# LepistaBioinformatics/classeq2

Hardware: AMD Instinct MI355X
Metric: query placements/sec, 10k-leaf tree, 150 bp reads (higher is better)
Workload: dtype u64

## Files before the change

classeq2_amd/csrc/cls_api.cpp:

```cpp
#include <hip/hip_runtime.h>
#include <ctype.h>
#include <stdio.h>
#include <stdlib.h>
#include <string.h>

#include <algorithm>
#include <mutex>
#include <new>
#include <string>
#include <thread>
#include <vector>

#include "cls_db.h"
#include "cls_device.h"
#include "cls_kernels.h"
#include "cls_place.h"
#include "cls_tuning.h"

namespace {

thread_local std::string g_err;

int fail(int code, const std::string& msg) {
    g_err = msg;
// ... 7 lines not shown
    } while (0)

struct Workspace {
    uint32_t* ptr = nullptr;
    uint64_t words = 0;
    hipEvent_t done = nullptr;
    hipStream_t stream = nullptr;
    uint64_t seq = 0;
    int launching = 0;
    bool busy = false;
    bool recorded = false;
};
struct TimedPair {
    hipEvent_t t0 = nullptr, t1 = nullptr;
    bool pending = false;
    bool in_use = false;
};
constexpr size_t MAX_WS_SLOTS = 8;
constexpr size_t MAX_TIMED_PAIRS = 256;

struct CallSlot {
    hipStream_t stream = nullptr;
    void *d_bases = nullptr, *d_off = nullptr, *d_out = nullptr, *d_stats = nullptr;
    uint64_t cap_bytes = 0;
    uint32_t cap_reads = 0, cap_stats = 0;
    bool busy = false;
};

cls::PlaceParams resolve(const cls_params* p) {
    cls::PlaceParams r;
    r.max_iterations = (p && (p->flags & CLS_HAS_MAX_ITERATIONS)) ? p->max_iterations : 1000;
    r.remove_intersection = (p && (p->flags & CLS_HAS_REMOVE_INTERSECTION)) ? (p->remove_intersection != 0) : 0;
    double c = 0.7;
    if (p && (p->flags & CLS_HAS_MIN_MATCH_COVERAGE)) {
        c = p->min_match_coverage;
        if (c > 1.0) c = 1.0; else if (c < 0.0) c = 0.0;
    }
    r.min_match_coverage = c;
    return r;
}

}

struct cls_db {
    int device = 0;
    int n_cu = 0;
    cls::DbDev dev{};
    cls_db_info info{};
    void* d_nodes = nullptr;
    void* d_kids = nullptr;
    void* d_table = nullptr;
    void* d_postings = nullptr;
    void* d_postings2 = nullptr;
    void* d_bucket_key = nullptr;
    void* d_mz_bucket = nullptr;
    void* d_direct = nullptr;
    void* d_direct16 = nullptr;
    void* d_sets = nullptr;
    void* d_sets2 = nullptr;
    std::mutex ws_mu;
    uint64_t max_read_len = 0;
    double kernel_ms_sum = 0.0;
    uint64_t kernel_launches = 0;
    std::vector<Workspace> ws;
    std::vector<TimedPair> timed;
    uint64_t ws_seq = 0;
    std::vector<CallSlot> calls;
};

namespace cls {
Tuning& tuning() {
    static Tuning t;
    return t;
}
}
namespace {
struct Knob { const char* name; int cls::Tuning::*field; };
const Knob KNOBS[] = {
    {"no_fast", &cls::Tuning::no_fast}, {"no_order", &cls::Tuning::no_order}, {"force_list", &cls::Tuning::force_list},
    {"no_mask_halves", &cls::Tuning::no_mask_halves}, {"no_fat_direct", &cls::Tuning::no_fat_direct}, {"no_tile", &cls::Tuning::no_tile}, {"tile_pass_codes", &cls::Tuning::tile_pass_codes}, {"tile_set_words", &cls::Tuning::tile_set_words}, {"time_class", &cls::Tuning::time_class}, {"tile_one_per_cu", &cls::Tuning::tile_one_per_cu}, {"tile_min_kmers", &cls::Tuning::tile_min_kmers}, {"no_tile_order", &cls::Tuning::no_tile_order}, {"tile_deal", &cls::Tuning::tile_deal}, {"blocks_per_cu", &cls::Tuning::blocks_per_cu}, {"key_blocks_per_cu", &cls::Tuning::key_blocks_per_cu},
    {"long_blocks_per_cu", &cls::Tuning::long_blocks_per_cu}, {"order_mode", &cls::Tuning::order_mode},
    {"order_windows", &cls::Tuning::order_windows}, {"order_both_strands", &cls::Tuning::order_both_strands},
    {"order_block_shift", &cls::Tuning::order_block_shift}, {"order_sample_shift", &cls::Tuning::order_sample_shift},
    {"profile_stop", &cls::Tuning::profile_stop}, {"timing", &cls::Tuning::timing},
};
}

extern "C" int cls_set_tuning(const char* name, int value) {
    if (!name) return fail(CLS_E_INVALID_ARG, "cls_set_tuning: null name");
    for (const Knob& k : KNOBS)
        if (strcmp(k.name, name) == 0) { cls::tuning().*(k.field) = value; return CLS_OK; }
    return fail(CLS_E_INVALID_ARG, std::string("cls_set_tuning: unknown knob ") + name);
}

extern "C" void cls_tuning_from_env(void) {
    for (const Knob& k : KNOBS) {
        std::string var = "CLS_";
        for (const char* c = k.name; *c; ++c) var += (char)toupper((unsigned char)*c);
        if (const char* v = getenv(var.c_str())) cls::tuning().*(k.field) = *v ? atoi(v) : 1;
    }
}

extern "C" const char* cls_last_error(void) { return g_err.c_str(); }
extern "C" void cls_internal_set_error(const char* msg) { g_err = msg ? msg : ""; }

extern "C" const char* cls_version(void) { return "classeq2_amd 0.1.0 gfx950 abi1"; }

extern "C" int cls_device_count(void) {
    int n = 0;
    if (hipGetDeviceCount(&n) != hipSuccess) return 0;
    return n;
}

extern "C" void cls_db_destroy(cls_db* db) {
    if (!db) return;
    int prev = 0;
    bool have_prev = hipGetDevice(&prev) == hipSuccess;
    (void)hipSetDevice(db->device);
    for (auto& w : db->ws) {
        if (w.done) { if (w.recorded) (void)hipEventSynchronize(w.done); (void)hipEventDestroy(w.done); }
        if (w.ptr) (void)hipFree(w.ptr);
    }
    for (auto& t : db->timed) {
        if (t.t0) (void)hipEventDestroy(t.t0);
        if (t.t1) (void)hipEventDestroy(t.t1);
    }
    for (auto& c : db->calls) {
        if (c.stream) { (void)hipStreamSynchronize(c.stream); (void)hipStreamDestroy(c.stream); }
        for (void* p : {c.d_bases, c.d_off, c.d_out, c.d_stats}) if (p) (void)hipFree(p);
    }
    if (db->d_nodes) (void)hipFree(db->d_nodes);
    if (db->d_kids) (void)hipFree(db->d_kids);
    if (db->d_table) (void)hipFree(db->d_table);
    if (db->d_postings) (void)hipFree(db->d_postings);
    if (db->d_postings2) (void)hipFree(db->d_postings2);
    if (db->d_bucket_key) (void)hipFree(db->d_bucket_key);
    if (db->d_mz_bucket) (void)hipFree(db->d_mz_bucket);
    if (db->d_direct) (void)hipFree(db->d_direct);
    if (db->d_direct16) (void)hipFree(db->d_direct16);
    if (db->d_sets) (void)hipFree(db->d_sets);
    if (db->d_sets2) (void)hipFree(db->d_sets2);
    if (have_prev) (void)hipSetDevice(prev);
    delete db;
}

static int encode(const cls_db_desc* d, cls::EncodedDb& E, const char* who) {
    std::string err;
    int rc = cls::encode_db(d, E, err);
    if (rc != CLS_OK) return fail(rc, std::string(who) + ": " + err);
    if (E.format == cls::FMT_LIST && E.postings.size() >= (1ULL << 32)) return fail(CLS_E_BAD_DB, std::string(who) + ": sorted-list postings exceed 2^32 words");
    return CLS_OK;
}

static int upload(const cls::EncodedDb& E, uint32_t n_buckets, int device, cls_db** out) {
    *out = nullptr;
    int n_dev = 0;
    if (hipGetDeviceCount(&n_dev) != hipSuccess || n_dev == 0)
        return fail(CLS_E_NO_DEVICE, "cls_db_create: no HIP device is visible (the placement path has no CPU fallback)");
    if (device < 0) CLS_HIP(hipGetDevice(&device));
    if (device >= n_dev) return fail(CLS_E_INVALID_ARG, "cls_db_create: device ordinal out of range");
    CLS_HIP(hipSetDevice(device));
    hipDeviceProp_t prop;
    CLS_HIP(hipGetDeviceProperties(&prop, device));
    cls_db* db = new cls_db();
    db->device = device;
    db->n_cu = prop.multiProcessorCount;
// ... 697 lines not shown
```

classeq2_amd/csrc/cls_devutil.h:

```cpp
#pragma once
#include <hip/hip_runtime.h>
#include <stdint.h>

#include "cls_device.h"
#include "cls_murmur.h"

namespace cls {
namespace {

__device__ __forceinline__ void wave_sync() {
    __builtin_amdgcn_fence(__ATOMIC_RELEASE, "wavefront");
    __builtin_amdgcn_wave_barrier();
    __builtin_amdgcn_fence(__ATOMIC_ACQUIRE, "wavefront");
}

__device__ __forceinline__ uint32_t uniform(uint32_t v) { return __builtin_amdgcn_readfirstlane(v); }

__device__ __forceinline__ uint32_t wave_sum(uint32_t v) {
    v += (uint32_t)__builtin_amdgcn_update_dpp(0, (int)v, 0xb1, 0xf, 0xf, true);
    v += (uint32_t)__builtin_amdgcn_update_dpp(0, (int)v, 0x4e, 0xf, 0xf, true);
    v += (uint32_t)__builtin_amdgcn_update_dpp(0, (int)v, 0x114, 0xf, 0xf, true);
    v += (uint32_t)__builtin_amdgcn_update_dpp(0, (int)v, 0x118, 0xf, 0xf, true);
    v += (uint32_t)__builtin_amdgcn_update_dpp(0, (int)v, 0x142, 0xa, 0xf, true);
    v += (uint32_t)__builtin_amdgcn_update_dpp(0, (int)v, 0x143, 0xc, 0xf, true);
    return (uint32_t)__builtin_amdgcn_readlane((int)v, 63);
}

struct snode_t { uint32_t s[8]; };
__device__ __forceinline__ snode_t load_node(const DNode* nodes, uint32_t row) {
    typedef __attribute__((address_space(4))) const uint32_t as4_u32;
    typedef __attribute__((address_space(4))) const char as4_char;
    as4_u32* p = (as4_u32*)((as4_char*)(uintptr_t)nodes + (uint32_t)(__builtin_amdgcn_readfirstlane(row) * (uint32_t)sizeof(DNode)));
    snode_t r;
#pragma unroll
    for (int i = 0; i < 8; ++i) r.s[i] = p[i];
    return r;
}

struct snode_pair_t { uint32_t s[16]; };
__device__ __forceinline__ snode_pair_t load_node_pair(const DNode* nodes, uint32_t row) {
    typedef __attribute__((address_space(4))) const uint32_t as4_u32;
    as4_u32* p = (as4_u32*)(uintptr_t)(nodes + __builtin_amdgcn_readfirstlane(row));
    snode_pair_t r;
#pragma unroll
    for (int i = 0; i < 16; ++i) r.s[i] = p[i];
    return r;
}

template <class T, bool ADDR32>
__device__ __forceinline__ T ldx(const void* base, uint32_t index) {
    if constexpr (ADDR32) return *reinterpret_cast<const T*>(reinterpret_cast<const char*>(base) + (uint32_t)(index * (uint32_t)sizeof(T)));
    else return reinterpret_cast<const T*>(base)[index];
}

template <bool ADDR32>
__device__ __forceinline__ uint2 ld_half(const uint32_t* half, uint32_t x, uint32_t right) {
    if constexpr (ADDR32) return ldx<uint2, true>(half, 2 * x + right);
    else return reinterpret_cast<const uint2*>(half)[2ull * x + right];
}

__device__ __forceinline__ uint64_t lds_u64(const uint8_t* p) { uint64_t v; __builtin_memcpy(&v, p, 8); return v; }
__device__ __forceinline__ uint64_t murmur3_h1_lds(const uint8_t* p, uint32_t len) {
    Mur3 m;
    const uint32_t nblocks = len >> 4;
#pragma unroll 1
    for (uint32_t b = 0; b < nblocks; ++b) m.block(lds_u64(p + 16 * b), lds_u64(p + 16 * b + 8));
    const uint32_t t = len & 15u;
    const uint8_t* tail = p + 16 * nblocks;
    uint64_t k1 = 0, k2 = 0;
    if (t > 0) { k1 = lds_u64(tail); if (t < 8) k1 &= (1ull << (8 * t)) - 1; }
    if (t > 8) { k2 = lds_u64(tail + 8) & ((1ull << (8 * (t - 8))) - 1); }
    return m.finish(k1, k2, t, len);
}

__device__ __forceinline__ uint32_t lds_prefix_code(const uint8_t* p, uint32_t m) {
    uint64_t x = (lds_u64(p) >> 1) & 0x0303030303030303ull;
    x = (x | (x >> 6)) & 0x000F000F000F000Full;
    x = (x | (x >> 12)) & 0x000000FF000000FFull;
    x = (x | (x >> 24)) & 0xFFFFull;
    return (uint32_t)x & ((1u << (2 * m)) - 1u);
}

__device__ __forceinline__ uint32_t mix32(uint32_t x) {
    x ^= x >> 16; x *= 0x7feb352du; x ^= x >> 15; x *= 0x846ca68bu; x ^= x >> 16;
    return x;
}

}
}
```

classeq2_amd/csrc/cls_kernels.hip:

```cpp
#include <hip/hip_runtime.h>
#include <stdlib.h>

#include <algorithm>
#include <type_traits>

#include "cls_device.h"
#include "cls_devutil.h"
#include "cls_kernels.h"
#include "cls_murmur.h"
#include "cls_sort.h"
#include "cls_tuning.h"

namespace cls {

namespace {

constexpr int WAVES_PER_BLOCK = 4;
#ifndef MIN_WAVES_PER_EU
#define MIN_WAVES_PER_EU 4
#endif
#ifndef FAST_MIN_WAVES
#define FAST_MIN_WAVES 5
#endif
#ifndef CLS_NARROW_CANON_BITS
// ... 1585 lines not shown
        const uint64_t b0 = have ? offsets[r] : 0, L64 = have ? offsets[r + 1] - b0 : 0;
        const bool keyed = have && L64 >= k && 2 * (L64 - k + 1) <= (uint64_t)key_cap;
        const uint32_t L = keyed ? (uint32_t)std::min<uint64_t>(L64, 64 + k - 1) : 0, nf = keyed ? L - k + 1 : 0;
        bool bad = false;
        for (uint32_t i = hl; i < L; i += 32) {
            uint8_t c = bases[b0 + i];
            if (c >= 'a' && c <= 'z') c -= 32;
            bad |= !(c == 'A' || c == 'C' || c == 'G' || c == 'T');
            ascii[i] = c;
        }
        const bool ok = keyed && half_of(__ballot(bad)) == 0;
        wave_sync();
        for (uint32_t w = hl; w < (L + 15) / 16 + 1; w += 32) {
            uint32_t acc = 0;
#pragma unroll
            for (int q = 0; q < 4; ++q) {
                uint32_t t = *reinterpret_cast<const uint32_t*>(ascii + 16 * w + 4 * q);
                t = (t >> 1) & 0x03030303u;
                t = (t | (t >> 6) | (t >> 12) | (t >> 18)) & 0xFFu;
                acc |= t << (8 * q);
            }
            if (w < WORDS) packed[w] = acc;
        }
        wave_sync();
        uint32_t e[2], hs[2];
#pragma unroll
        for (int s = 0; s < 2; ++s) {
            const uint32_t p = hl + 32 * s;
            const bool valid = ok && p < nf;
            const uint32_t w = valid ? p >> 4 : 0, sh = valid ? (2 * p) & 31 : 0;
            const uint32_t d0 = packed[w], d1 = packed[w + 1];
            uint32_t code = (uint32_t)((((uint64_t)d1 << 32) | d0) >> sh) & kmask;
            uint32_t rcc = __builtin_bitreverse32(code ^ (0xAAAAAAAAu & kmask));
            rcc = ((rcc >> 1) & 0x55555555u) | ((rcc & 0x55555555u) << 1);
            rcc >>= (32 - 2 * k);
            code = rcc < code ? rcc : code;
            const uint32_t v = ldx<uint32_t, ADDR32>(direct, valid ? code : 0u);
            e[s] = valid ? v : 0u;
            hs[s] = mix32(code);
        }
        uint32_t cand = 0, n_cand = 0;
        for (uint32_t tier = 0; tier < 4; ++tier) {
            const bool need = n_cand < 4;
            uint32_t c_new = 0, n_new = 0;
#pragma unroll
            for (int s = 0; s < 2; ++s) {
                const bool c = (e[s] & SET_ID_MASK) != 0 && (e[s] >> TIER_SHIFT) <= tier;
                c_new |= (c ? 1u : 0u) << s;
                n_new += (uint32_t)__popc(half_of(__ballot(c)));
            }
            if (need) { cand = c_new; n_cand = n_new; }
            if (__ballot(n_cand < 4) == 0) break;
        }
        uint32_t rank = n_cand >> 1, prefix = 0;
        for (int bit = (int)db.set_bits - 1; bit >= 0; --bit) {
            uint32_t c0 = 0;
#pragma unroll
            for (int s = 0; s < 2; ++s) {
                const uint32_t t = e[s] & SET_ID_MASK;
                const bool z = ((cand >> s) & 1u) && ((t ^ prefix) >> (bit + 1)) == 0 && !((t >> bit) & 1u);
                c0 += (uint32_t)__popc(half_of(__ballot(z)));
            }
            if (rank >= c0) { rank -= c0; prefix |= 1u << bit; }
        }
        uint32_t mh = 0xFFFFFFFFu, mha = 0xFFFFFFFFu;
#pragma unroll
        for (int s = 0; s < 2; ++s) {
            if ((cand >> s) & 1u) mh = hs[s] < mh ? hs[s] : mh;
            if ((e[s] & SET_ID_MASK) != 0) mha = hs[s] < mha ? hs[s] : mha;
        }
        for (int o = 16; o > 0; o >>= 1) {
            const uint32_t o1 = __shfl_xor(mh, o), o2 = __shfl_xor(mha, o);
            mh = o1 < mh ? o1 : mh;
            mha = o2 < mha ? o2 : mha;
        }
        if (have && hl == 0) {
            keys[r] = (ok && n_cand) ? make_order_key(key_mode, prefix, mh, mha, block_shift, db.set_bits) : ~0ull;
            idx[r] = r;
        }
        wave_sync();
    }
}

constexpr int LONG_THREADS = 256;
constexpr int LONG_STATE_WORDS = 5;

constexpr uint32_t LONG_LDS_ARITY = 256;
struct LongSh {
    uint32_t acc[4];
    unsigned long long acc64;
    uint32_t n_next;
    uint32_t n_pass, n_best, best_row;
    int32_t best_diff, best_one, best_rest;
    uint32_t cpre[LONG_LDS_ARITY + 1];
    uint32_t cnt_l[LONG_LDS_ARITY], only_l[LONG_LDS_ARITY];
};

__device__ __forceinline__ uint32_t append_slot(bool keep, uint32_t* counter) {
    const uint32_t lane = threadIdx.x & 63;
    const uint64_t m = __ballot(keep);
    if (!m) return 0;
    const int leader = __ffsll((unsigned long long)m) - 1;
    uint32_t base = 0;
    if ((int)lane == leader) base = atomicAdd(counter, (uint32_t)__popcll(m));
    base = __shfl(base, leader);
    return base + (uint32_t)__popcll(m & ((1ull << lane) - 1));
}

template <int N>
__device__ __forceinline__ void long_sum(uint32_t (&v)[N], LongSh& sh) {
    __syncthreads();
    if (threadIdx.x < N) sh.acc[threadIdx.x] = 0;
    __syncthreads();
#pragma unroll
    for (int i = 0; i < N; ++i) {
        const uint32_t w = wave_sum(v[i]);
        if ((threadIdx.x & 63) == 0 && w) atomicAdd(&sh.acc[i], w);
    }
    __syncthreads();
#pragma unroll
    for (int i = 0; i < N; ++i) v[i] = sh.acc[i];
}

template <bool SPLIT, bool STATS>
__global__ __launch_bounds__(LONG_THREADS) void place_long_kernel(DbDev db, PlaceParams prm, const uint8_t* __restrict__ bases,
                                                                  const uint64_t* __restrict__ offsets,
                                                                  const uint32_t* __restrict__ list,
                                                                  const uint32_t* __restrict__ list_len,
                                                                  cls_placement* __restrict__ out, cls_query_stats* __restrict__ stats,
                                                                  uint32_t* __restrict__ ws, uint64_t ws_stride_words, uint32_t cap,
                                                                  uint32_t set_size, uint32_t arity_pad) {
    __shared__ LongSh sh;
    constexpr uint32_t NT = LONG_THREADS;
    const uint32_t tid = threadIdx.x, lane = tid & 63;
    uint32_t* const buf0 = ws + (size_t)blockIdx.x * ws_stride_words;
    uint32_t* const buf1 = buf0 + (size_t)LONG_STATE_WORDS * cap;
    uint32_t* const cnt = buf1 + (size_t)LONG_STATE_WORDS * cap;
    uint32_t* const only = cnt + arity_pad;
    uint32_t* const set = buf1;
    uint32_t* const ent = buf0 + 4 * (size_t)cap;
    const DNode* __restrict__ nodes = db.nodes;
    const uint32_t* __restrict__ post = db.postings;
    const uint4* __restrict__ recs = reinterpret_cast<const uint4*>(db.postings);
    const uint32_t k = db.k, m_eff = db.m_eff;
    const bool rm = prm.remove_intersection != 0;
    const uint32_t n_list = *list_len;
    for (uint32_t li = blockIdx.x; li < n_list; li += gridDim.x) {
        __syncthreads();
        const uint32_t r = list[li];
        const uint64_t b0 = offsets[r], L64 = offsets[r + 1] - b0;
        auto put_stats = [&](uint32_t nk_, uint32_t nm, uint32_t nr, uint64_t lp) {
            if (STATS && stats && tid == 0) {
                uint64_t* s = reinterpret_cast<uint64_t*>(stats + r);
                s[0] = (uint64_t)nk_ | ((uint64_t)nm << 32);
                s[1] = (uint64_t)nr;
                s[2] = lp;
            }
        };
        auto record = [&](uint32_t status, int32_t one, int32_t rest, uint32_t levels, uint64_t clade) {
            if (tid == 0) {
                uint64_t* o = reinterpret_cast<uint64_t*>(out + r);
                o[0] = (uint64_t)(status & 0xFF) | ((uint64_t)(uint32_t)one << 32);
                o[1] = (uint64_t)(uint32_t)rest | ((uint64_t)levels << 32);
                o[2] = clade;
            }
        };
// ... 263 lines not shown
                            st[0] = lo; st[1] = hi; st[2] = vlo; st[3] = vhi; st[4] = cur[4 * (size_t)cap + j];
                        }
                    }
                }
                const uint32_t p = append_slot(keep, &sh.n_next);
                if (keep) {
#pragma unroll
                    for (int i = 0; i < (SPLIT ? 3 : LONG_STATE_WORDS); ++i) nxt[(size_t)i * cap + p] = st[i];
                }
            }
            __syncthreads();
            n_act = sh.n_next;
            { uint32_t* t = cur; cur = nxt; nxt = t; }
            prow = best_row;
        }
    }
}

constexpr int CLASSIFY_THREADS = 256, CLASSIFY_PER_THREAD = 4;
struct ClassCaps { uint32_t cap[N_LISTS]; };
__global__ __launch_bounds__(CLASSIFY_THREADS) void classify_kernel(const uint64_t* __restrict__ offsets, const uint32_t* __restrict__ order, uint32_t n_reads, uint32_t k, ClassCaps caps,
                                                                   uint32_t* __restrict__ lists, uint32_t* __restrict__ counts,
                                                                   cls_placement* __restrict__ out, cls_query_stats* __restrict__ stats) {
    __shared__ uint32_t s_cnt[N_LISTS], s_base[N_LISTS];
    if (threadIdx.x < N_LISTS) s_cnt[threadIdx.x] = 0;
    __syncthreads();
    const uint32_t lane = threadIdx.x & 63;
    const uint32_t first = blockIdx.x * (CLASSIFY_THREADS * CLASSIFY_PER_THREAD) + threadIdx.x;
    int cls_id[CLASSIFY_PER_THREAD];
    uint32_t pos[CLASSIFY_PER_THREAD], rd[CLASSIFY_PER_THREAD];
#pragma unroll
    for (int i = 0; i < CLASSIFY_PER_THREAD; ++i) {
        const uint32_t at = first + i * CLASSIFY_THREADS;
        const uint32_t r = (order && at < n_reads) ? order[at] : at;
        rd[i] = r;
        cls_id[i] = -1;
        pos[i] = 0;
        if (at < n_reads) {
            const uint64_t L = offsets[r + 1] - offsets[r];
            const uint64_t nk = L < k ? 0 : 2 * (L - k + 1);
#pragma unroll
            for (int c = N_LISTS - 1; c >= 0; --c) if (nk <= caps.cap[c]) cls_id[i] = c;
            if (cls_id[i] < 0) {
                uint64_t* o = reinterpret_cast<uint64_t*>(out + r);
                o[0] = CLS_ERR_READ_TOO_LONG; o[1] = 0; o[2] = 0;
                if (stats) {
                    uint64_t* st = reinterpret_cast<uint64_t*>(stats + r);
                    st[0] = nk > 0xFFFFFFFFull ? 0xFFFFFFFFull : nk; st[1] = 0; st[2] = 0;
                }
            }
        }
#pragma unroll
        for (int c = 0; c < N_LISTS; ++c) {
            const uint64_t m = __ballot(cls_id[i] == c);
            if (!m) continue;
            uint32_t base = 0;
            if (lane == 0) base = atomicAdd(&s_cnt[c], (uint32_t)__popcll(m));
            base = __shfl(base, 0);
            if (cls_id[i] == c) pos[i] = base + (uint32_t)__popcll(m & ((1ull << lane) - 1));
        }
    }
    __syncthreads();
    if (threadIdx.x < N_LISTS) s_base[threadIdx.x] = s_cnt[threadIdx.x] ? atomicAdd(&counts[threadIdx.x], s_cnt[threadIdx.x]) : 0u;
    __syncthreads();
#pragma unroll
    for (int i = 0; i < CLASSIFY_PER_THREAD; ++i) {
        const int c = cls_id[i];
        if (c >= 0) lists[(size_t)c * n_reads + s_base[c] + pos[i]] = rd[i];
    }
}

}

namespace {
constexpr int N_CLASSES = 2;
constexpr int BLK_WAVES = 8, BLK_SLOTS = 16, BLK_SET_BITS = 14;
constexpr int ORDER_KEY_BITS_MAX = TIER_SHIFT + 20;
int order_key_bits(const DbDev& db) {
    const Tuning& tn = tuning();
    const int bits = tn.order_mode == 1 ? (int)db.set_bits + 20 : std::max(1, (int)db.set_bits - tn.order_block_shift) + 16;
    return std::min<int>(64, bits + 1);
}
constexpr int CLS_SLOTS[N_CLASSES] = {5, 16};
constexpr int CLS_SET_BITS[N_CLASSES] = {9, 11};
constexpr int NARROW_CANON_BITS = CLS_NARROW_CANON_BITS;

bool use_fast(const DbDev& db);
bool use_order(const DbDev& db, uint32_t n_reads) {
    return use_fast(db) && !tuning().no_order && n_reads >= 4096;
}
bool use_fast(const DbDev& db) {
    const bool front = db.direct != nullptr || (db.addr32 && db.k <= 256);
    return db.format == FMT_SPLIT && (db.binary_tree || db.max_nonleaf_arity <= FAST_MAX_ARITY) && front && !tuning().no_fast;
}
int fast_mode(const DbDev& db) { return db.direct == nullptr ? 2 : (db.direct16 && db.addr32) ? (db.canonical ? 4 : 3) : db.canonical ? 1 : 0; }
bool mode_canonical(int mode) { return mode == 1 || mode == 4; }
int set_bits_of(const DbDev& db, int c) { return (c == 0 && use_fast(db) && mode_canonical(fast_mode(db))) ? NARROW_CANON_BITS : CLS_SET_BITS[c]; }
uint32_t seq_cap_of(const DbDev& db, int c) { return (2 * (64 * CLS_SLOTS[c] / 2 + db.k) + 15) & ~15u; }
uint32_t ascii_cap_of(const DbDev& db, int c) {
    const uint32_t fwd = 64 * CLS_SLOTS[c] / 2 + db.k + 16;
    return ((db.direct ? fwd : 2 * fwd) + 15) & ~15u;
}
uint32_t child_ws_stride(const DbDev& db);
constexpr uint32_t CHILD_LDS_MAX = 256;
bool child_in_lds(const DbDev& db) { return child_ws_stride(db) != 0 && child_ws_stride(db) <= CHILD_LDS_MAX; }
size_t smem_of(const DbDev& db, int c) {
    if (use_fast(db)) {
        const uint32_t ac = ascii_cap_of(db, c);
        const uint32_t packed = db.direct ? 4u * (((ac >> 4) + 2 + 3) & ~3u) : 0u;
        return (size_t)WAVES_PER_BLOCK * (ac + packed + (12u << set_bits_of(db, c)) + (db.binary_tree ? 0u : 12u * FAST_MAX_ARITY + 16u));
    }
    return (size_t)WAVES_PER_BLOCK * (seq_cap_of(db, c) + (4u << CLS_SET_BITS[c]) + 4u * 64 * CLS_SLOTS[c]) +
           (child_in_lds(db) ? (size_t)WAVES_PER_BLOCK * 2 * child_ws_stride(db) * 4 : 0);
}

using FastFn = decltype(place_fast_kernel<CLS_SLOTS[0], CLS_SET_BITS[0], false, false, 0, false>);
using SplitFn = decltype(place_split_kernel<CLS_SLOTS[0], CLS_SET_BITS[0], false, false>);
using WaveFn = decltype(place_wave_kernel<CLS_SLOTS[0], CLS_SET_BITS[0], false, false>);
struct ClassKernel {
    FastFn* fast;
    SplitFn* split;
    WaveFn* wave;
    size_t smem;
    std::string name;
    const void* fn() const { return fast ? (const void*)fast : split ? (const void*)split : (const void*)wave; }
};
template <int SLOTS, int SET_BITS>
ClassKernel class_kernel_t(const DbDev& db, int c, bool stats) {
    const size_t smem = smem_of(db, c);
    auto fast = [&](auto... v) { return ClassKernel{place_fast_kernel<decltype(v)::value...>, nullptr, nullptr, smem, instance_name("place_fast_kernel", v...)}; };
    auto split = [&](auto... v) { return ClassKernel{nullptr, place_split_kernel<decltype(v)::value...>, nullptr, smem, instance_name("place_split_kernel", v...)}; };
    auto wave = [&](auto... v) { return ClassKernel{nullptr, nullptr, place_wave_kernel<decltype(v)::value...>, smem, instance_name("place_wave_kernel", v...)}; };
    const Int<SLOTS> sl;
    const Int<SET_BITS> sb;
    return with_bool(stats, [&](auto st) {
        if (use_fast(db)) {
            return with_bool(!db.binary_tree, [&](auto poly) {
                const std::true_type addr32;
                switch (fast_mode(db)) {
                    case 2: return fast(sl, sb, st, addr32, Int<2>{}, poly);
                    case 3: return fast(sl, sb, st, addr32, Int<3>{}, poly);
                    case 4: return fast(sl, sb, st, addr32, Int<4>{}, poly);
                }
                return with_bool(db.addr32, [&](auto a32) { return fast_mode(db) == 1 ? fast(sl, sb, st, a32, Int<1>{}, poly) : fast(sl, sb, st, a32, Int<0>{}, poly); });
            });
        }
        if (db.format == FMT_SPLIT) return with_bool(!db.binary_tree, [&](auto poly) { return split(sl, sb, st, poly); });
        return with_bool(db.max_nonleaf_arity <= 2, [&](auto binary) { return wave(sl, sb, st, binary); });
    });
}
ClassKernel class_kernel(const DbDev& db, int c, bool stats) {
    if (c == 1) return class_kernel_t<CLS_SLOTS[1], CLS_SET_BITS[1]>(db, 1, stats);
    if (set_bits_of(db, 0) != CLS_SET_BITS[0]) return class_kernel_t<CLS_SLOTS[0], NARROW_CANON_BITS>(db, 0, stats);
    return class_kernel_t<CLS_SLOTS[0], CLS_SET_BITS[0]>(db, 0, stats);
}

uint32_t child_ws_stride(const DbDev& db) {
    if (db.format == FMT_SPLIT) return db.binary_tree ? 0u : ((std::max(db.max_nonleaf_arity, 1u) + 63) & ~63u);
    return db.max_nonleaf_arity <= 2 ? 0u : ((db.max_nonleaf_arity + 63) & ~63u);
}
uint32_t blk_seq_cap(const DbDev& db) { return (2 * (64 * BLK_WAVES * BLK_SLOTS / 2 + db.k) + 15) & ~15u; }
auto block_kernel(const DbDev& db, bool stats) {
    const size_t smem = (size_t)blk_seq_cap(db) + (4u << BLK_SET_BITS) + 4u * 64 * BLK_WAVES * BLK_SLOTS + 64 +
                        (child_in_lds(db) ? (size_t)2 * child_ws_stride(db) * 4 : 0);
    auto inst = [&](auto... v) { return pick(place_block_kernel<decltype(v)::value...>, smem, "place_block_kernel", v...); };
    const bool split = db.format == FMT_SPLIT, binary = split ? db.binary_tree != 0 : db.max_nonleaf_arity <= 2;
    return with_bool(stats, [&](auto st) { return with_bool(binary, [&](auto bi) { return with_bool(split, [&](auto sp) {
        return inst(Int<BLK_WAVES>{}, Int<BLK_SLOTS>{}, Int<BLK_SET_BITS>{}, st, bi, sp);
    }); }); });
}
auto long_kernel(const DbDev& db, bool stats) {
    auto inst = [&](auto... v) { return pick(place_long_kernel<decltype(v)::value...>, 0, "place_long_kernel", v...); };
    return with_bool(db.format == FMT_SPLIT, [&](auto sp) { return with_bool(stats, [&](auto st) { return inst(sp, st); }); });
}

using KeyFn = decltype(order_key_kernel<2, true, true, false>);
using KeyHalfFn = decltype(order_key_half_kernel<true>);
struct KeyKernel {
    KeyFn* full;
    KeyHalfFn* half;
    size_t smem;
    std::string name;
    const void* fn() const { return full ? (const void*)full : (const void*)half; }
};
KeyKernel key_kernel(const DbDev& db, bool sizing) {
    const Tuning& tn = tuning();
    const bool fwd = !tn.order_both_strands, hashed = fast_mode(db) == 2;
    if (!sizing && !hashed && fwd && tn.order_windows == 64 && (uint32_t)tn.order_sample_shift >= 32)
        return with_bool(db.addr32, [&](auto a32) { return KeyKernel{nullptr, order_key_half_kernel<decltype(a32)::value>, 0, instance_name("order_key_half_kernel", a32)}; });
    const uint32_t ac = ascii_cap_of(db, 0);
    const size_t smem = (size_t)WAVES_PER_BLOCK * (ac + (db.direct ? 4u * (((ac >> 4) + 2 + 3) & ~3u) : 0u) + 16u);
    auto inst = [&](auto... v) { return KeyKernel{order_key_kernel<decltype(v)::value...>, nullptr, smem, instance_name("order_key_kernel", v...)}; };
    auto of = [&](auto a32, auto hs) {
        if (fwd && tn.order_windows <= 64) return inst(Int<2>{}, a32, std::true_type{}, hs);
        if (fwd || sizing) return inst(Int<CLS_SLOTS[0]>{}, a32, std::true_type{}, hs);
        return inst(Int<CLS_SLOTS[0]>{}, a32, std::false_type{}, hs);
    };
    if (hashed) return of(std::true_type{}, std::true_type{});
    return db.addr32 ? of(std::true_type{}, std::false_type{}) : of(std::false_type{}, std::false_type{});
}
}

void PlacePlan::class_caps(uint32_t (&cap)[N_LISTS]) const {
    for (uint32_t& c : cap) c = 0;
    cap[0] = (uint32_t)(64 * CLS_SLOTS[0]);
    if (max_kmers > cap[0]) cap[1] = (uint32_t)(64 * CLS_SLOTS[1]);
    if (max_kmers > (uint32_t)(64 * CLS_SLOTS[1])) cap[2] = tiled ? tile_from : (uint32_t)(64 * BLK_WAVES * BLK_SLOTS);
    if (tiled) {
        for (uint32_t i = 0; i < tile.n_sub; ++i) cap[3 + i] = tile.sub[i].cap_kmers;
        cap[6] = tile.whole.cap_kmers;
    }
    cap[7] = long_cap;
}

std::string PlacePlan::class_kernel_name(const DbDev& db, int c, bool stats) const {
    if (c < 2) return class_kernel(db, c, stats).name;
    if (c == 2) return block_kernel(db, stats).name;
    if (c < 6) return tile_kernel_name(db, stats, tile.sub[c - 3]);
    if (c == 6) return tile_kernel_name(db, stats, tile.whole);
    return long_kernel(db, stats).name;
}

PlacePlan plan_place(const DbDev& db, uint32_t n_reads, uint32_t n_cu, bool stats, uint32_t long_cap, uint32_t n_long) {
    PlacePlan p{};
    const int forced = tuning().blocks_per_cu;
    const uint32_t want = (n_reads + WAVES_PER_BLOCK - 1) / WAVES_PER_BLOCK;
    uint64_t child_words = 0;
    for (int c = 0; c < N_CLASSES; ++c) {
        int per_cu = forced;
        const ClassKernel k = class_kernel(db, c, stats);
        if (per_cu <= 0 && (hipOccupancyMaxActiveBlocksPerMultiprocessor(&per_cu, k.fn(), 64 * WAVES_PER_BLOCK, k.smem) != hipSuccess || per_cu <= 0))
            per_cu = 1;
        uint32_t cap = n_cu * (uint32_t)per_cu;
        if (child_ws_stride(db) && !child_in_lds(db)) {
            const uint64_t per_block = (uint64_t)WAVES_PER_BLOCK * 2 * child_ws_stride(db) * 4;
            const uint64_t fit = std::max<uint64_t>(1, (128ull << 20) / per_block);
            if (cap > fit) cap = (uint32_t)fit;
        }
        p.grid[c] = want < cap ? (want ? want : 1) : cap;
        if (!child_in_lds(db)) child_words = std::max<uint64_t>(child_words, (uint64_t)p.grid[c] * WAVES_PER_BLOCK * 2 * child_ws_stride(db));
    }
    p.grid_blk = std::max<uint32_t>(1, std::min<uint32_t>(n_reads, n_cu));
    if (!child_in_lds(db)) child_words = std::max<uint64_t>(child_words, (uint64_t)p.grid_blk * 2 * child_ws_stride(db));
    p.ordered = use_order(db, n_reads);
    uint64_t w = 16 + (uint64_t)N_LISTS * n_reads;
    w += w & 1;
    if (p.ordered) {
        p.grid[0] = std::max<uint32_t>(8, p.grid[0] & ~7u);
        p.grid[1] = std::max<uint32_t>(8, p.grid[1] & ~7u);
        {
            int per_cu = tuning().key_blocks_per_cu;
            const KeyKernel k = key_kernel(db, true);
            if (per_cu <= 0 && (hipOccupancyMaxActiveBlocksPerMultiprocessor(&per_cu, k.fn(), 64 * WAVES_PER_BLOCK, k.smem) != hipSuccess || per_cu <= 0)) per_cu = 4;
            if (tuning().key_blocks_per_cu <= 0 && fast_mode(db) == 2) per_cu *= 2;
            p.grid_key = std::max<uint32_t>(1, std::min<uint32_t>(want, n_cu * (uint32_t)per_cu));
        }
        p.keys_off_words = w;
        w += 6 * (uint64_t)n_reads;
        p.sort_off_words = w;
        p.sort_bytes = order_temp_bytes(n_reads);
        w += (p.sort_bytes + 3) / 4 + 2;
        w += w & 1;
    }
    p.child_off_words = w;
    w += child_words;
    w += w & 1;
    p.max_kmers = n_long ? std::max<uint32_t>(long_cap, 2u) : MAX_READ_KMERS;
    const uint32_t blk_cap = (uint32_t)(64 * BLK_WAVES * BLK_SLOTS);
    p.tile_from = blk_cap;
    if (tile_usable(db)) {
        p.tile_from = tuning().tile_min_kmers > 0 ? std::min<uint32_t>(blk_cap, (uint32_t)tuning().tile_min_kmers) : (uint32_t)(64 * CLS_SLOTS[1]);
        if (p.max_kmers > p.tile_from) {
            p.tile = tile_plan(db, stats, p.tile_from, p.max_kmers, n_reads, n_cu);
            p.tiled = p.tile.whole.cap_kmers > p.tile_from;
        }
    }
    if (p.tiled) {
        p.tile_off_words = w;
        w += p.tile.scratch_words;
        w += w & 1;
    } else p.tile_from = blk_cap;
    if (p.max_kmers > MAX_READ_KMERS || p.tiled) {
        long_cap = p.max_kmers;
        p.long_cap = long_cap;
        p.long_set = 1;
        while (p.long_set < 2 * (uint64_t)long_cap) p.long_set <<= 1;
        p.long_arity = (std::max(db.max_nonleaf_arity, 1u) + 63) & ~63u;
        p.long_stride_words = 2 * (uint64_t)LONG_STATE_WORDS * long_cap + 2 * (uint64_t)p.long_arity;
        const uint64_t fit = std::max<uint64_t>(1, (2ull << 30) / (p.long_stride_words * 4));
        const uint64_t per_cu_long = (uint64_t)std::max(1, tuning().long_blocks_per_cu);
        p.grid_long = (uint32_t)std::min<uint64_t>({(uint64_t)std::max<uint32_t>(1u, n_long ? n_long : n_reads), (uint64_t)n_cu * per_cu_long, fit});
        if (p.tiled && p.tile.whole.cap_kmers >= long_cap) p.grid_long = std::min<uint32_t>(p.grid_long, 8u);
        p.long_off_words = w;
        w += p.long_stride_words * p.grid_long;
    }
    p.ws_bytes = w * 4;
    p.blk = p.max_kmers > (uint32_t)(64 * CLS_SLOTS[1]) && (!p.tiled || p.tile_from > (uint32_t)(64 * CLS_SLOTS[1]));
    const bool gene = tuning().time_class == 2;
    p.timed = p.tiled && (p.max_kmers > MAX_READ_KMERS || gene) ? PlacePlan::TIME_TILE : p.blk && gene ? PlacePlan::TIME_BLOCK : PlacePlan::TIME_CLASS0;
    p.timed_name = p.timed == PlacePlan::TIME_TILE ? p.tile.name : p.timed == PlacePlan::TIME_BLOCK ? block_kernel(db, stats).name : class_kernel(db, 0, stats).name;
    return p;
}

hipError_t launch_place(const DbDev& db, const PlaceParams& prm, const PlacePlan& plan, const uint8_t* d_bases,
                        const uint64_t* d_offsets, uint32_t n_reads, cls_placement* d_out, cls_query_stats* d_stats,
                        uint32_t* d_ws, hipStream_t stream, hipEvent_t ev_start, hipEvent_t ev_stop) {
    if (n_reads == 0) return hipSuccess;
    uint32_t* counts = d_ws;
    uint32_t* lists[N_LISTS];
    for (int c = 0; c < N_LISTS; ++c) lists[c] = d_ws + 16 + (size_t)c * n_reads;
    uint32_t* child_ws = (child_ws_stride(db) && !child_in_lds(db)) ? d_ws + plan.child_off_words : nullptr;
    hipError_t e = hipMemsetAsync(counts, 0, 64, stream);
    if (e != hipSuccess) return e;
    const uint32_t profile_stop = (uint32_t)tuning().profile_stop;
    const uint32_t ws_stride = child_ws_stride(db);
    const bool st = d_stats != nullptr;
    auto classify = [&](const uint32_t* order) {
        ClassCaps caps{};
        plan.class_caps(caps.cap);
        return launch_kernel(classify_kernel, dim3((n_reads + CLASSIFY_THREADS * CLASSIFY_PER_THREAD - 1) / (CLASSIFY_THREADS * CLASSIFY_PER_THREAD)), dim3(CLASSIFY_THREADS), 0,
                             stream, d_offsets, order, n_reads, db.k, caps, lists[0], counts, d_out, d_stats);
    };
    const uint32_t* list0 = lists[0];
    uint32_t list0_n = 0, xcd_chunks = 0;
    if (!plan.ordered) e = classify(nullptr);
    else {
        uint64_t* keys_in = reinterpret_cast<uint64_t*>(d_ws + plan.keys_off_words);
        uint64_t* keys_out = keys_in + n_reads;
        uint32_t* idx_in = reinterpret_cast<uint32_t*>(keys_out + n_reads);
        uint32_t* idx_out = idx_in + n_reads;
        const Tuning& tn = tuning();
        const uint32_t key_mode = (uint32_t)tn.order_mode;
        const uint32_t block_shift = (uint32_t)tn.order_block_shift;
        const uint32_t key_cap = (plan.tiled && !tn.no_tile_order) ? 0xFFFFFFFFu : (uint32_t)(64 * CLS_SLOTS[1]);
        const KeyKernel k = key_kernel(db, false);
        const dim3 block(64 * WAVES_PER_BLOCK);
        if (k.half) {
            const uint32_t grid_half = std::max<uint32_t>(1, std::min<uint32_t>((n_reads + 2 * WAVES_PER_BLOCK - 1) / (2 * WAVES_PER_BLOCK), plan.grid_key));
            e = launch_kernel(k.half, dim3(grid_half), block, k.smem, stream, db, d_bases, d_offsets, n_reads, keys_in, idx_in, key_mode, block_shift, key_cap);
        } else {
            e = launch_kernel(k.full, dim3(plan.grid_key), block, k.smem, stream, db, d_bases, d_offsets, n_reads, keys_in, idx_in, ascii_cap_of(db, 0), key_mode,
                              block_shift, (uint32_t)tn.order_sample_shift, tn.order_both_strands ? 0u : 1u, key_cap);
        }
        if (e != hipSuccess) return e;
        e = order_reads(d_ws + plan.sort_off_words, keys_in, idx_out, n_reads, order_key_bits(db) - 1, stream);
        if (e != hipSuccess) return e;
        list0 = idx_out;
        list0_n = n_reads;
        xcd_chunks = 1;
        e = classify(idx_out);
    }
    if (e != hipSuccess) return e;
    auto launch_class = [&](int c) {
        const ClassKernel k = class_kernel(db, c, st);
        const dim3 grid(plan.grid[c]), block(64 * WAVES_PER_BLOCK);
        if (k.fast) {
            return launch_kernel(k.fast, grid, block, k.smem, stream, db, prm, d_bases, d_offsets, xcd_chunks ? list0 : lists[c], counts + c, list0_n, xcd_chunks,
                                 d_out, d_stats, ascii_cap_of(db, c), profile_stop);
        }
        if (k.split)
            return launch_kernel(k.split, grid, block, k.smem, stream, db, prm, d_bases, d_offsets, lists[c], counts + c, d_out, d_stats, seq_cap_of(db, c),
                                 profile_stop, child_ws, ws_stride);
        return launch_kernel(k.wave, grid, block, k.smem, stream, db, prm, d_bases, d_offsets, lists[c], counts + c, d_out, d_stats, seq_cap_of(db, c), child_ws,
                             ws_stride);
    };
    auto timed = [&](PlacePlan::Timed t, auto&& launch) {
        if (ev_start && plan.timed == t) (void)hipEventRecord(ev_start, stream);
        const hipError_t r = launch();
        if (ev_stop && plan.timed == t) (void)hipEventRecord(ev_stop, stream);
        return r;
    };
    e = timed(PlacePlan::TIME_CLASS0, [&] { return launch_class(0); });
    if (e != hipSuccess) return e;
    if (plan.max_kmers > (uint32_t)(64 * CLS_SLOTS[0])) {
        e = launch_class(1);
        if (e != hipSuccess) return e;
    }
    if (plan.blk) {
        const auto k = block_kernel(db, st);
        e = timed(PlacePlan::TIME_BLOCK, [&] {
            return launch_kernel(k.fn, dim3(plan.grid_blk), dim3(64 * BLK_WAVES), k.smem, stream, db, prm, d_bases, d_offsets, lists[2], counts + 2, d_out, d_stats,
                                 blk_seq_cap(db), child_ws, ws_stride);
        });
        if (e != hipSuccess) return e;
    }
    if (plan.tiled) {
        const uint32_t* sub_lists[TILE_MAX_SUB] = {lists[3], lists[4], lists[5]};
        const uint32_t* sub_lens[TILE_MAX_SUB] = {counts + 3, counts + 4, counts + 5};
        e = timed(PlacePlan::TIME_TILE, [&] {
            return tile_launch(db, prm, plan.tile, st, d_bases, d_offsets, sub_lists, sub_lens, lists[6], counts + 6, d_out, d_stats, lists[7], counts + 7,
                               d_ws + plan.tile_off_words, plan.ordered && !tuning().no_tile_order, stream);
        });
        if (e != hipSuccess) return e;
    }
    if (plan.grid_long) {
        const auto k = long_kernel(db, st);
        e = launch_kernel(k.fn, dim3(plan.grid_long), dim3(LONG_THREADS), k.smem, stream, db, prm, d_bases, d_offsets, lists[7], counts + 7, d_out, d_stats,
                          d_ws + plan.long_off_words, plan.long_stride_words, plan.long_cap, (uint32_t)plan.long_set, plan.long_arity);
    }
    return e;
}

}
```

classeq2_amd/csrc/cls_tuning.h:

```cpp
#pragma once

namespace cls {

struct Tuning {
    int no_fast = 0;
    int no_order = 0;
    int force_list = 0;
    int no_mask_halves = 0;
    int no_fat_direct = 0;
    int no_tile = 0;
    int tile_pass_codes = 0;
    int tile_set_words = 0;
    int tile_min_kmers = 0;
    int tile_deal = 64;
    int no_tile_order = 0;
    int tile_one_per_cu = 0;
    int time_class = 0;
    int blocks_per_cu = 0;
    int key_blocks_per_cu = 0;
    int long_blocks_per_cu = 2;
    int order_mode = 0;
    int order_windows = 64;
    int order_both_strands = 0;
    int order_block_shift = 2;
    int order_sample_shift = 32;
    int profile_stop = 0;
    int timing = 0;
};

Tuning& tuning();

}
```

Baseline: 157.7 million.

## Add bottom-k hash-sampled order-key kernel with four reads per wave

Adds a new order-key kernel that packs each read into shared memory with one read per 16-lane quarter-wave. It hashes every canonical k-mer window with an invertible mix and selects the n smallest hashes (bottom-k, default 16) by repeated row-level DPP min reductions. Only the sampled k-mers are looked up in the direct table, and the codes are recovered with unmix32, so fewer random table gathers are needed per read and four reads share each wave. Sort keys now come from a sample, which may change read ordering and locality in the classify stage. The sampling loop adds serial reduction work per read.

```diff
diff --git a/classeq2_amd/csrc/cls_api.cpp b/classeq2_amd/csrc/cls_api.cpp
--- a/classeq2_amd/csrc/cls_api.cpp
+++ b/classeq2_amd/csrc/cls_api.cpp
@@ -113,6 +113,7 @@
     {"long_blocks_per_cu", &cls::Tuning::long_blocks_per_cu}, {"order_mode", &cls::Tuning::order_mode},
     {"order_windows", &cls::Tuning::order_windows}, {"order_both_strands", &cls::Tuning::order_both_strands},
     {"order_block_shift", &cls::Tuning::order_block_shift}, {"order_sample_shift", &cls::Tuning::order_sample_shift},
+    {"order_sample", &cls::Tuning::order_sample},
     {"profile_stop", &cls::Tuning::profile_stop}, {"timing", &cls::Tuning::timing},
 };
 }
diff --git a/classeq2_amd/csrc/cls_devutil.h b/classeq2_amd/csrc/cls_devutil.h
--- a/classeq2_amd/csrc/cls_devutil.h
+++ b/classeq2_amd/csrc/cls_devutil.h
@@ -24,6 +24,13 @@
     v += (uint32_t)__builtin_amdgcn_update_dpp(0, (int)v, 0x142, 0xa, 0xf, true);
     v += (uint32_t)__builtin_amdgcn_update_dpp(0, (int)v, 0x143, 0xc, 0xf, true);
     return (uint32_t)__builtin_amdgcn_readlane((int)v, 63);
+}
+
+__device__ __forceinline__ uint32_t row16_min(uint32_t v) {
+    v = min(v, (uint32_t)__builtin_amdgcn_update_dpp(0, (int)v, 0xB1, 0xF, 0xF, false));
+    v = min(v, (uint32_t)__builtin_amdgcn_update_dpp(0, (int)v, 0x4E, 0xF, 0xF, false));
+    v = min(v, (uint32_t)__builtin_amdgcn_update_dpp(0, (int)v, 0x141, 0xF, 0xF, false));
+    return min(v, (uint32_t)__builtin_amdgcn_update_dpp(0, (int)v, 0x140, 0xF, 0xF, false));
 }
 
 struct snode_t { uint32_t s[8]; };
@@ -85,6 +92,10 @@
     x ^= x >> 16; x *= 0x7feb352du; x ^= x >> 15; x *= 0x846ca68bu; x ^= x >> 16;
     return x;
 }
+__device__ __forceinline__ uint32_t unmix32(uint32_t x) {
+    x ^= x >> 16; x *= 0x43021123u; x ^= (x >> 15) ^ (x >> 30); x *= 0x1d69e2a5u; x ^= x >> 16;
+    return x;
+}
 
 }
 }
diff --git a/classeq2_amd/csrc/cls_kernels.hip b/classeq2_amd/csrc/cls_kernels.hip
--- a/classeq2_amd/csrc/cls_kernels.hip
+++ b/classeq2_amd/csrc/cls_kernels.hip
@@ -1691,6 +1691,148 @@
     }
 }
 
+constexpr uint32_t SAMPLE_MAX_WINDOWS = 160;
+constexpr uint32_t SAMPLE_MAX = 64;
+__device__ __forceinline__ uint32_t nonzero_bytes(uint32_t v) { return (((v & 0x7F7F7F7Fu) + 0x7F7F7F7Fu) | v) & 0x80808080u; }
+template <bool ADDR32>
+__global__ __launch_bounds__(64 * WAVES_PER_BLOCK) void order_key_sample_kernel(DbDev db, const uint8_t* __restrict__ bases,
+                                                                              const uint64_t* __restrict__ offsets, uint32_t n_reads,
+                                                                              uint64_t* __restrict__ keys, uint32_t* __restrict__ idx,
+                                                                              uint32_t key_mode, uint32_t block_shift, uint32_t key_cap,
+                                                                              uint32_t n_sample) {
+    constexpr uint32_t PER = SAMPLE_MAX_WINDOWS / 16;
+    constexpr uint32_t SL = SAMPLE_MAX / 16;
+    constexpr uint32_t MAXL = SAMPLE_MAX_WINDOWS + DIRECT_MAX_K - 1;
+    constexpr uint32_t WORDS = (MAXL + 15) / 16 + 1;
+    static_assert(WORDS <= 16 && SAMPLE_MAX_WINDOWS % 16 == 0 && SAMPLE_MAX % 16 == 0, "one packed word per lane");
+    __shared__ uint32_t s_packed[WAVES_PER_BLOCK * 4][WORDS];
+    const uint32_t wave = threadIdx.x >> 6, lane = threadIdx.x & 63, quarter = lane >> 4, ql = lane & 15;
+    uint32_t* packed = s_packed[wave * 4 + quarter];
+    const uint32_t k = db.k;
+    const uint32_t kmask = (1u << (2 * k)) - 1u;
+    const uint32_t* __restrict__ direct = db.direct;
+    const uint32_t r_first = (blockIdx.x * WAVES_PER_BLOCK + wave) * 4, stride = gridDim.x * WAVES_PER_BLOCK * 4;
+    auto mine = [&](uint64_t m) { return (uint32_t)(m >> (16 * quarter)) & 0xFFFFu; };
+    auto canon_at = [&](uint32_t p) {
+        const uint32_t w = p >> 4, sh = (2 * p) & 31;
+        const uint32_t code = (uint32_t)((((uint64_t)packed[w + 1] << 32) | packed[w]) >> sh) & kmask;
+        uint32_t rcc = __builtin_bitreverse32(code ^ (0xAAAAAAAAu & kmask));
+        rcc = ((rcc >> 1) & 0x55555555u) | ((rcc & 0x55555555u) << 1);
+        rcc >>= (32 - 2 * k);
+        return rcc < code ? rcc : code;
+    };
+    for (uint32_t r0 = r_first; r0 < n_reads; r0 += stride) {
+        const uint32_t r = r0 + quarter;
+        const bool have = r < n_reads;
+        const uint64_t b0 = have ? offsets[r] : 0, L64 = have ? offsets[r + 1] - b0 : 0;
+        const bool keyed = have && L64 >= k && 2 * (L64 - k + 1) <= (uint64_t)key_cap;
+        const bool sampled = keyed && L64 - k + 1 <= SAMPLE_MAX_WINDOWS;
+        const uint32_t nf = keyed ? (sampled ? (uint32_t)(L64 - k + 1) : 64u) : 0u, L = keyed ? nf + k - 1 : 0u;
+        bool bad = false;
+        if (keyed && ql < (L + 15) / 16 + 1) {
+            const uint8_t* p = bases + b0 + 16 * ql;
+            const uintptr_t a = (uintptr_t)p & ~(uintptr_t)3, end = (uintptr_t)(bases + b0 + L);
+            const uint32_t sh = 8u * ((uint32_t)(uintptr_t)p & 3u);
+            uint32_t d[5];
+#pragma unroll
+            for (int i = 0; i < 5; ++i) d[i] = a + 4 * i < end ? *reinterpret_cast<const uint32_t*>(a + 4 * i) : 0u;
+            uint32_t acc = 0;
+#pragma unroll
+            for (int q = 0; q < 4; ++q) {
+                uint32_t t = (uint32_t)((((uint64_t)d[q + 1] << 32) | d[q]) >> sh);
+                const int left = (int)L - (int)(16 * ql + 4 * q);
+                const uint32_t in = left >= 4 ? 0xFFFFFFFFu : left <= 0 ? 0u : (1u << (8 * left)) - 1u;
+                const uint32_t lc = t | 0x20202020u;
+                bad |= (nonzero_bytes(lc ^ 0x61616161u) & nonzero_bytes(lc ^ 0x63636363u) & nonzero_bytes(lc ^ 0x67676767u) &
+                        nonzero_bytes(lc ^ 0x74747474u) & in) != 0;
+                t = (t >> 1) & 0x03030303u;
+                t = (t | (t >> 6) | (t >> 12) | (t >> 18)) & 0xFFu;
+                acc |= t << (8 * q);
+            }
+            packed[ql] = acc;
+        }
+        const bool ok = keyed && mine(__ballot(bad)) == 0;
+        wave_sync();
+        uint32_t pick[SL];
+#pragma unroll
+        for (int s = 0; s < (int)SL; ++s) pick[s] = 0xFFFFFFFFu;
+        const bool any_sampled = __ballot(ok && sampled) != 0;
+        if (any_sampled) {
+            uint32_t h[PER];
+#pragma unroll
+            for (int j = 0; j < (int)PER; ++j) {
+                const uint32_t p = ql + 16 * j;
+                const bool valid = ok && sampled && p < nf;
+                h[j] = valid ? mix32(canon_at(valid ? p : 0u)) : 0xFFFFFFFFu;
+            }
+            uint32_t lo = 0;
+            for (uint32_t i = 0; i < n_sample; ++i) {
+                uint32_t m = 0xFFFFFFFFu;
+#pragma unroll
+                for (int j = 0; j < (int)PER; ++j) m = min(m, h[j] >= lo ? h[j] : 0xFFFFFFFFu);
+                m = row16_min(m);
+#pragma unroll
+                for (int s = 0; s < (int)SL; ++s)
+                    if (i == 16 * s + ql) pick[s] = m;
+                lo = m == 0xFFFFFFFFu ? m : m + 1;
+                if (__ballot(m != 0xFFFFFFFFu) == 0) break;
+            }
+        }
+        const uint32_t n_slots = __ballot(ok && !sampled) ? SL : (n_sample + 15) / 16;
+        uint32_t e[SL], hs[SL];
+#pragma unroll
+        for (int s = 0; s < (int)SL; ++s) {
+            e[s] = 0;
+            hs[s] = 0xFFFFFFFFu;
+            if ((uint32_t)s >= n_slots) continue;
+            const uint32_t p = ql + 16 * s;
+            const bool valid = ok && (sampled ? pick[s] != 0xFFFFFFFFu : p < nf);
+            const uint32_t code = sampled ? unmix32(pick[s]) : canon_at(valid ? p : 0u);
+            hs[s] = sampled ? pick[s] : mix32(code);
+            if (valid) e[s] = ldx<uint32_t, ADDR32>(direct, code);
+        }
+        uint32_t cand = 0, n_cand = 0;
+        for (uint32_t tier = 0; tier < 4; ++tier) {
+            const bool need = n_cand < 4;
+            uint32_t c_new = 0, n_new = 0;
+#pragma unroll
+            for (int s = 0; s < (int)SL; ++s) {
+                if ((uint32_t)s >= n_slots) continue;
+                const bool c = (e[s] & SET_ID_MASK) != 0 && (e[s] >> TIER_SHIFT) <= tier;
+                c_new |= (c ? 1u : 0u) << s;
+                n_new += (uint32_t)__popc(mine(__ballot(c)));
+            }
+            if (need) { cand = c_new; n_cand = n_new; }
+            if (__ballot(n_cand < 4) == 0) break;
+        }
+        uint32_t rank = n_cand >> 1, prefix = 0;
+        for (int bit = (int)db.set_bits - 1; bit >= 0; --bit) {
+            uint32_t c0 = 0;
+#pragma unroll
+            for (int s = 0; s < (int)SL; ++s) {
+                if ((uint32_t)s >= n_slots) continue;
+                const uint32_t t = e[s] & SET_ID_MASK;
+                const bool z = ((cand >> s) & 1u) && ((t ^ prefix) >> (bit + 1)) == 0 && !((t >> bit) & 1u);
+                c0 += (uint32_t)__popc(mine(__ballot(z)));
+            }
+            if (rank >= c0) { rank -= c0; prefix |= 1u << bit; }
+        }
+        uint32_t mh = 0xFFFFFFFFu, mha = 0xFFFFFFFFu;
+#pragma unroll
+        for (int s = 0; s < (int)SL; ++s) {
+            if ((cand >> s) & 1u) mh = hs[s] < mh ? hs[s] : mh;
+            if ((e[s] & SET_ID_MASK) != 0) mha = hs[s] < mha ? hs[s] : mha;
+        }
+        mh = row16_min(mh);
+        mha = row16_min(mha);
+        if (have && ql == 0) {
+            keys[r] = (ok && n_cand) ? make_order_key(key_mode, prefix, mh, mha, block_shift, db.set_bits) : ~0ull;
+            idx[r] = r;
+        }
+        wave_sync();
+    }
+}
+
 constexpr int LONG_THREADS = 256;
 constexpr int LONG_STATE_WORDS = 5;
 
@@ -2120,6 +2262,7 @@
     return std::min<int>(64, bits + 1);
 }
 constexpr int CLS_SLOTS[N_CLASSES] = {5, 16};
+static_assert(SAMPLE_MAX_WINDOWS == 64 * CLS_SLOTS[0] / 2, "the sampled key covers the class-0 reads");
 constexpr int CLS_SET_BITS[N_CLASSES] = {9, 11};
 constexpr int NARROW_CANON_BITS = CLS_NARROW_CANON_BITS;
 
@@ -2214,21 +2357,26 @@
 
 using KeyFn = decltype(order_key_kernel<2, true, true, false>);
 using KeyHalfFn = decltype(order_key_half_kernel<true>);
+using KeySampleFn = decltype(order_key_sample_kernel<true>);
 struct KeyKernel {
     KeyFn* full;
     KeyHalfFn* half;
+    KeySampleFn* sample;
     size_t smem;
     std::string name;
-    const void* fn() const { return full ? (const void*)full : (const void*)half; }
+    const void* fn() const { return full ? (const void*)full : half ? (const void*)half : (const void*)sample; }
 };
 KeyKernel key_kernel(const DbDev& db, bool sizing) {
     const Tuning& tn = tuning();
     const bool fwd = !tn.order_both_strands, hashed = fast_mode(db) == 2;
-    if (!sizing && !hashed && fwd && tn.order_windows == 64 && (uint32_t)tn.order_sample_shift >= 32)
-        return with_bool(db.addr32, [&](auto a32) { return KeyKernel{nullptr, order_key_half_kernel<decltype(a32)::value>, 0, instance_name("order_key_half_kernel", a32)}; });
+    const bool fast_knobs = !hashed && fwd && tn.order_windows == 64 && (uint32_t)tn.order_sample_shift >= 32;
+    if (fast_knobs && tn.order_sample > 0)
+        return with_bool(db.addr32, [&](auto a32) { return KeyKernel{nullptr, nullptr, order_key_sample_kernel<decltype(a32)::value>, 0, instance_name("order_key_sample_kernel", a32)}; });
+    if (!sizing && fast_knobs)
+        return with_bool(db.addr32, [&](auto a32) { return KeyKernel{nullptr, order_key_half_kernel<decltype(a32)::value>, nullptr, 0, instance_name("order_key_half_kernel", a32)}; });
     const uint32_t ac = ascii_cap_of(db, 0);
     const size_t smem = (size_t)WAVES_PER_BLOCK * (ac + (db.direct ? 4u * (((ac >> 4) + 2 + 3) & ~3u) : 0u) + 16u);
-    auto inst = [&](auto... v) { return KeyKernel{order_key_kernel<decltype(v)::value...>, nullptr, smem, instance_name("order_key_kernel", v...)}; };
+    auto inst = [&](auto... v) { return KeyKernel{order_key_kernel<decltype(v)::value...>, nullptr, nullptr, smem, instance_name("order_key_kernel", v...)}; };
     auto of = [&](auto a32, auto hs) {
         if (fwd && tn.order_windows <= 64) return inst(Int<2>{}, a32, std::true_type{}, hs);
         if (fwd || sizing) return inst(Int<CLS_SLOTS[0]>{}, a32, std::true_type{}, hs);
@@ -2373,7 +2521,12 @@
         const uint32_t key_cap = (plan.tiled && !tn.no_tile_order) ? 0xFFFFFFFFu : (uint32_t)(64 * CLS_SLOTS[1]);
         const KeyKernel k = key_kernel(db, false);
         const dim3 block(64 * WAVES_PER_BLOCK);
-        if (k.half) {
+        if (k.sample) {
+            const uint32_t grid_sample = std::max<uint32_t>(1, std::min<uint32_t>((n_reads + 4 * WAVES_PER_BLOCK - 1) / (4 * WAVES_PER_BLOCK), plan.grid_key));
+            const uint32_t n_sample = std::min<uint32_t>((uint32_t)tn.order_sample, SAMPLE_MAX);
+            e = launch_kernel(k.sample, dim3(grid_sample), block, k.smem, stream, db, d_bases, d_offsets, n_reads, keys_in, idx_in, key_mode, block_shift, key_cap,
+                              n_sample);
+        } else if (k.half) {
             const uint32_t grid_half = std::max<uint32_t>(1, std::min<uint32_t>((n_reads + 2 * WAVES_PER_BLOCK - 1) / (2 * WAVES_PER_BLOCK), plan.grid_key));
             e = launch_kernel(k.half, dim3(grid_half), block, k.smem, stream, db, d_bases, d_offsets, n_reads, keys_in, idx_in, key_mode, block_shift, key_cap);
         } else {
diff --git a/classeq2_amd/csrc/cls_tuning.h b/classeq2_amd/csrc/cls_tuning.h
--- a/classeq2_amd/csrc/cls_tuning.h
+++ b/classeq2_amd/csrc/cls_tuning.h
@@ -24,6 +24,7 @@
     int order_both_strands = 0;
     int order_block_shift = 2;
     int order_sample_shift = 32;
+    int order_sample = 16;
     int profile_stop = 0;
     int timing = 0;
 };
```

Result: faster. 159.7 million, median of 6 (+1.2%).
